# idonahum/photoVerse

Hardware: AMD Instinct MI355X
Metric: denoising steps/sec at 512x512 bs=16, 50-step loop (2 UNet fwd + CFG + DPM-Solver++ step per step) (higher is better)
Workload: dtype f16; 1 GPU; configs[1] shape timed over 96 steps instead of 50: SD-v1.5 UNet + PhotoVerse processors, 96-step loop, bs=16/GPU, 512x512 (64x64 latents), P=1, guidance 7.5, fp16; per_gpu_batch=16, global_batch=16, latent=64, parallelism=dp1 (batch-sharded, 1 all_gather), hip_graph=True, graph_branches=2

## Files before the change

### photoverse_amd/csrc/pv_gemm.hip

```cpp
#include "pv_gemm_dev.h"

namespace {

constexpr int BK = 64;
constexpr int ROW_BYTES = BK * 2;

template <int NF, int MIV = 4>
struct TileCfg {
    static constexpr int MI = MIV;
    static constexpr int BM = 2 * MI * 16;
    static constexpr int BN = NF * 32;
    static constexpr int NWAVES = 4;
    static constexpr int THREADS = NWAVES * 64;
    static constexpr int A_PER_WAVE = BM / 8 / NWAVES;
    static constexpr int STAGES = 2;
    static constexpr int A_BYTES = BM * ROW_BYTES;
    static constexpr int B_BYTES = BN * ROW_BYTES;
    static constexpr int STAGE_BYTES = A_BYTES + B_BYTES;
    static constexpr int SMEM_BYTES = STAGES * STAGE_BYTES;
    static constexpr int B_PIECES = NF * 4;
    static constexpr int B_PER_WAVE = (B_PIECES + NWAVES - 1) / NWAVES;
};

__device__ __forceinline__ float epi_act(float x, int act) {
    if (act == PV_ACT_SILU) return pv_silu(x);
    if (act == PV_ACT_QUICK_GELU) return pv_quick_gelu(x);
    if (act == PV_ACT_LEAKY_RELU) return x > 0.f ? x : 0.01f * x;
    return x;
}

__device__ __forceinline__ half8_t lds_frag(const char* base, int row, int chunk) {
    return *reinterpret_cast<const half8_t*>(base + row * ROW_BYTES + ((chunk ^ (row & 7)) << 4));
}

template <int N>
__device__ __forceinline__ void wait_vmcnt() {
    static_assert(N >= 0 && N < 64, "vmcnt is a 6-bit field");
    asm volatile("s_waitcnt vmcnt(%0)" ::"n"(N) : "memory");
}


__device__ __forceinline__ float row16_sum(float v) {
    v += __builtin_bit_cast(float, __builtin_amdgcn_update_dpp(0, __builtin_bit_cast(int, v), 0x128, 0xf, 0xf, false));
    v += __builtin_bit_cast(float, __builtin_amdgcn_update_dpp(0, __builtin_bit_cast(int, v), 0x124, 0xf, 0xf, false));
    v += __builtin_bit_cast(float, __builtin_amdgcn_update_dpp(0, __builtin_bit_cast(int, v), 0x122, 0xf, 0xf, false));
    v += __builtin_bit_cast(float, __builtin_amdgcn_update_dpp(0, __builtin_bit_cast(int, v), 0x121, 0xf, 0xf, false));
    return v;
}

template <int NF, bool CONV, bool GEGLU, bool CS = false, bool MULTI = false, int MIV = 4>
__global__ __launch_bounds__(256, MIV == 4 ? 2 : 3) void gemm_conv_kernel(const pv_gemm_params_dev p, const int tiles_n,
                                                                              const int nblk, const int order, const int tpw_arg) {
    const int tpw = MULTI ? tpw_arg : 1;
    using Cfg = TileCfg<NF, MIV>;
    static_assert(MIV == 4 || (!CS && !MULTI && !CONV), "the 64-row tile exists for plain Linear layers only");
    constexpr int BM = Cfg::BM;
    constexpr int NW = Cfg::NWAVES;
    constexpr int MI = Cfg::MI;
    constexpr int AP = Cfg::A_PER_WAVE;
    extern __shared__ __attribute__((aligned(16))) char smem[];

    const int lane = pv_lane_id();
    const int wave = pv_wave_id();
    const int bid = (order & 2) ? (int)blockIdx.x : pv_xcd_remap((int)blockIdx.x, nblk);
    const int m_fast = order & 1;
    const int tiles_m = nblk / tiles_n;
    const int tile_m = m_fast ? bid % tiles_m : bid / tiles_n;
    const int tile_n = (m_fast ? bid / tiles_m : bid % tiles_n) * tpw;
    const int m0 = tile_m * BM;
    int n0 = tile_n * Cfg::BN;

    const int cin = p.c0 + p.c1;
    const int K = p.taps * cin;
    const int nk_total = K / BK;
    const int nk_per = (nk_total + (int)gridDim.y - 1) / (int)gridDim.y;
    const int k_begin = (int)blockIdx.y * nk_per;
    const int nk = max(0, min(nk_total, k_begin + nk_per) - k_begin);

    const int lrow = lane >> 3;
    const int src_chunk = (lane & 7) ^ lrow;
    const int lane_cc2 = src_chunk * 16;
    constexpr unsigned OOB = 0x80000000u;
    const __amdgpu_buffer_rsrc_t ra0 = __builtin_amdgcn_make_buffer_rsrc(const_cast<void*>(p.a0), 0, (int)p.a0_bytes, 0x00020000);
    const __amdgpu_buffer_rsrc_t ra1 = __builtin_amdgcn_make_buffer_rsrc(const_cast<void*>(p.a1 ? p.a1 : p.a0), 0, (int)p.a1_bytes, 0x00020000);
    const __amdgpu_buffer_rsrc_t rw = __builtin_amdgcn_make_buffer_rsrc(const_cast<void*>(p.w), 0, (int)p.w_bytes, 0x00020000);
    const int hw_out = p.hout * p.wout;
    const bool fast_conv = CONV && p.stride == 1 && !p.upsample;
    const int hl = p.upsample ? p.hin * 2 : p.hin;
    const int wl = p.upsample ? p.win * 2 : p.win;
    unsigned a_off0[AP], a_off1[AP];
    unsigned a_mask[AP];
    int a_b[AP], a_y[AP], a_x[AP];
#pragma unroll
    for (int i = 0; i < AP; ++i) {
        const int m = m0 + (wave + i * NW) * 8 + lrow;
        const bool ok = m < p.M;
        if (CONV) {
            const int b = m / hw_out;
            const int rem = m - b * hw_out;
            const int y = rem / p.wout, x = rem - y * p.wout;
            a_b[i] = b; a_y[i] = y * p.stride + 1 - p.pad; a_x[i] = x * p.stride + 1 - p.pad;
            unsigned mask = 0;
#pragma unroll
            for (int t = 0; t < 9; ++t) {
                const int iy = a_y[i] + t / 3 - 1, ix = a_x[i] + t % 3 - 1;
                if (ok && iy >= 0 && iy < hl && ix >= 0 && ix < wl) mask |= 1u << t;
            }
            a_mask[i] = mask;
            const unsigned pix = (unsigned)((b * p.hin + y) * p.win + x);
            a_off0[i] = pix * (unsigned)(p.lda0 * 2) + lane_cc2;
            a_off1[i] = pix * (unsigned)(p.lda1 * 2) + lane_cc2;
        } else {
            a_mask[i] = ok ? 1u : 0u;
            a_off0[i] = ok ? (unsigned)m * (unsigned)(p.lda0 * 2) + lane_cc2 : OOB;
            a_off1[i] = ok ? (unsigned)m * (unsigned)(p.lda1 * 2) + lane_cc2 : OOB;
            a_b[i] = a_y[i] = a_x[i] = 0;
        }
    }
    unsigned w_off[Cfg::B_PER_WAVE];
#pragma unroll
    for (int i = 0; i < Cfg::B_PER_WAVE; ++i) {
        const int n = n0 + min(wave + i * NW, Cfg::B_PIECES - 1) * 8 + lrow;
        w_off[i] = (unsigned)n * (unsigned)(K * 2) + lane_cc2;
    }
    const bool b_full = (Cfg::B_PIECES % NW == 0) || (wave + (Cfg::B_PER_WAVE - 1) * NW < Cfg::B_PIECES);

    auto stage = [&](int g_local, int buf) {
        const int tn = g_local / nk;
        const int kt = k_begin + (g_local - tn * nk);
        char* sa = smem + buf * Cfg::STAGE_BYTES;
        char* sb = sa + Cfg::A_BYTES;
        const int chunk = CONV ? kt / 9 : kt;
        const int tap = CONV ? kt - chunk * 9 : 0;
        const int c = chunk * BK;
        const bool first = c < p.c0;
        const __amdgpu_buffer_rsrc_t ra = first ? ra0 : ra1;
        const int ld2 = (first ? p.lda0 : p.lda1) * 2;
        const int sc2 = (first ? c : c - p.c0) * 2;
        const int ky = tap / 3, kx = tap - ky * 3;
        const int tap_delta = ((ky - 1) * p.win + (kx - 1)) * ld2 + sc2;
#pragma unroll
        for (int i = 0; i < AP; ++i) {
            unsigned off;
            if (!CONV) {
                off = (first ? a_off0[i] : a_off1[i]) + (unsigned)sc2;
            } else if (fast_conv) {
                off = ((a_mask[i] >> tap) & 1u) ? (first ? a_off0[i] : a_off1[i]) + (unsigned)tap_delta : OOB;
            } else {
                const int iy = a_y[i] + ky - 1, ix = a_x[i] + kx - 1;
                const int py = p.upsample ? iy >> 1 : iy, px = p.upsample ? ix >> 1 : ix;
                const unsigned pix = (unsigned)((a_b[i] * p.hin + py) * p.win + px);
                off = ((a_mask[i] >> tap) & 1u) ? pix * (unsigned)ld2 + (unsigned)(sc2 + lane_cc2) : OOB;
            }
            __builtin_amdgcn_raw_ptr_buffer_load_lds(ra, PV_LDS_PTR(sa + (wave + i * NW) * 8 * ROW_BYTES), 16, (int)off, 0, 0, 0);
        }
        const unsigned wk2 = (unsigned)(tap * cin + c) * 2u + (unsigned)tn * (unsigned)(Cfg::BN * K * 2);
#pragma unroll
        for (int i = 0; i < Cfg::B_PER_WAVE; ++i) {
            if (i < Cfg::B_PER_WAVE - 1 || b_full)
                __builtin_amdgcn_raw_ptr_buffer_load_lds(rw, PV_LDS_PTR(sb + (wave + i * NW) * 8 * ROW_BYTES), 16, (int)(w_off[i] + wk2), 0, 0, 0);
        }
    };

    float4_t acc[NF][MI];
#pragma unroll
    for (int ni = 0; ni < NF; ++ni)
#pragma unroll
        for (int mi = 0; mi < MI; ++mi) acc[ni][mi] = float4_t{0.f, 0.f, 0.f, 0.f};

    const int wm = wave >> 1, wn = wave & 1;
    const int fr = lane & 15, fq = lane >> 4;

    constexpr int S = Cfg::STAGES;
    auto read_half = [&](half8_t (&xa)[MI], half8_t (&wb)[NF], int kt, int ks) {
        const char* sa = smem + (kt % S) * Cfg::STAGE_BYTES;
        const char* sb = sa + Cfg::A_BYTES;
#pragma unroll
        for (int mi = 0; mi < MI; ++mi) xa[mi] = lds_frag(sa, wm * (MI * 16) + mi * 16 + fr, ks * 4 + fq);
#pragma unroll
        for (int ni = 0; ni < NF; ++ni) wb[ni] = lds_frag(sb, wn * (NF * 16) + ni * 16 + fr, ks * 4 + fq);
    };
    auto mma_half = [&](const half8_t (&xa)[MI], const half8_t (&wb)[NF]) {
#pragma unroll
        for (int ni = 0; ni < NF; ++ni)
#pragma unroll
            for (int mi = 0; mi < MI; ++mi)
                acc[ni][mi] = __builtin_amdgcn_mfma_f32_16x16x32_f16(wb[ni], xa[mi], acc[ni][mi], 0, 0, 0);
    };

    const int T = nk * tpw;
#pragma unroll
    for (int s = 0; s < S; ++s)
        if (s < T) stage(s, s);
    if (T >= S && S == 3) {
        if (b_full) wait_vmcnt<(AP + Cfg::B_PER_WAVE) * 2>(); else wait_vmcnt<(AP + Cfg::B_PER_WAVE - 1) * 2>();
    } else if (T >= S && S == 2) {
        if (b_full) wait_vmcnt<(AP + Cfg::B_PER_WAVE)>(); else wait_vmcnt<(AP + Cfg::B_PER_WAVE - 1)>();
    } else {
        wait_vmcnt<0>();
    }
    __builtin_amdgcn_s_barrier();
    asm volatile("" ::: "memory");

    half8_t xa0[MI], wb0[NF], xa1[MI], wb1[NF];
    if (T > 0) read_half(xa0, wb0, 0, 0);
    for (int tn = 0; tn < tpw; ++tn) {
    for (int kt = 0; kt < nk; ++kt) {
        const int g = tn * nk + kt;
        read_half(xa1, wb1, g, 1);
        __builtin_amdgcn_sched_barrier(0);
        mma_half(xa0, wb0);
        __builtin_amdgcn_sched_barrier(0);
        if (g + 1 < T) {
            if (S == 3 && g + S - 1 < T) {
                if (b_full) wait_vmcnt<(AP + Cfg::B_PER_WAVE)>(); else wait_vmcnt<(AP + Cfg::B_PER_WAVE - 1)>();
            } else {
                wait_vmcnt<0>();
            }
            asm volatile("s_waitcnt lgkmcnt(0)" ::: "memory");
            __builtin_amdgcn_s_barrier();
            asm volatile("" ::: "memory");
            if (g + S < T) stage(g + S, g % S);
            __builtin_amdgcn_sched_barrier(0);
            if (kt + 1 < nk) {
                read_half(xa0, wb0, g + 1, 0);
                __builtin_amdgcn_sched_barrier(0);
            }
        }
        mma_half(xa1, wb1);
        __builtin_amdgcn_sched_barrier(0);
    }

    if (gridDim.y > 1) {
        float* slab = p.splitk_ws + (size_t)blockIdx.y * p.M * p.N;
#pragma unroll
        for (int mi = 0; mi < MI; ++mi) {
            const int m = m0 + wm * (MI * 16) + mi * 16 + fr;
            if (m >= p.M) continue;
#pragma unroll
            for (int ni = 0; ni < NF; ++ni) {
                const int n = n0 + wn * (NF * 16) + ni * 16 + fq * 4;
                *reinterpret_cast<float4_t*>(slab + (size_t)m * p.N + n) = acc[ni][mi];
            }
        }
        return;
    }
    const int nbase = n0 + wn * (NF * 16) + fq * 4;
    if (GEGLU) {
        float4_t bv[NF / 2], bg[NF / 2];
#pragma unroll
        for (int q = 0; q < NF / 2; ++q) {
            bv[q] = p.bias ? *reinterpret_cast<const float4_t*>(p.bias + nbase + (2 * q) * 16) : float4_t{0.f, 0.f, 0.f, 0.f};
            bg[q] = p.bias ? *reinterpret_cast<const float4_t*>(p.bias + nbase + (2 * q + 1) * 16) : float4_t{0.f, 0.f, 0.f, 0.f};
        }
#pragma unroll
        for (int mi = 0; mi < MI; ++mi) {
            const int m = m0 + wm * (MI * 16) + mi * 16 + fr;
            if (m >= p.M) continue;
            unsigned pk[NF / 2][2];
#pragma unroll
            for (int q = 0; q < NF / 2; ++q) {
                const float4_t v = acc[2 * q][mi] + bv[q], g = acc[2 * q + 1][mi] + bg[q];
                pk[q][0] = __builtin_bit_cast(unsigned, half2_t{(half_t)(v[0] * pv_gelu_erf(g[0])), (half_t)(v[1] * pv_gelu_erf(g[1]))});
                pk[q][1] = __builtin_bit_cast(unsigned, half2_t{(half_t)(v[2] * pv_gelu_erf(g[2])), (half_t)(v[3] * pv_gelu_erf(g[3]))});
            }
            half_t* orow = reinterpret_cast<half_t*>(p.out) + (size_t)m * p.ldc + (n0 >> 1) + wn * (NF * 8);
            static_assert(!GEGLU || NF == 4, "GEGLU epilogue pairs the two value|gate fragment pairs of a wave");
            {
                const auto r0 = __builtin_amdgcn_permlane16_swap(pk[0][0], pk[1][0], false, false);
                const auto r1 = __builtin_amdgcn_permlane16_swap(pk[0][1], pk[1][1], false, false);
                const unsigned a0 = r0[0], b0 = r0[1], a1 = r1[0], b1 = r1[1];
                const int col = (fq & 1) ? 16 + (fq - 1) * 4 : fq * 4;
                typedef unsigned uint4_t __attribute__((ext_vector_type(4)));
                *reinterpret_cast<uint4_t*>(orow + col) = uint4_t{a0, a1, b0, b1};
            }
        }
    } else {
        float4_t bias_v[NF];
#pragma unroll
        for (int ni = 0; ni < NF; ++ni)
            bias_v[ni] = p.bias ? *reinterpret_cast<const float4_t*>(p.bias + nbase + ni * 16) : float4_t{0.f, 0.f, 0.f, 0.f};
        constexpr int RB = MULTI ? 2 : MI;
        half4_t res[NF][MI];
        if (p.residual && !MULTI) {
#pragma unroll
            for (int mi = 0; mi < MI; ++mi) {
                const int m = min(m0 + wm * (MI * 16) + mi * 16 + fr, p.M - 1);
#pragma unroll
                for (int ni = 0; ni < NF; ++ni)
                    res[ni][mi] = *reinterpret_cast<const half4_t*>(reinterpret_cast<const half_t*>(p.residual) + (size_t)m * p.ldr + nbase + ni * 16);
            }
        }
        const bool want_cs = CS && p.colstats != nullptr && !p.out_f32;
        float4_t cs[NF], cq[NF];
#pragma unroll
        for (int ni = 0; ni < NF; ++ni) cs[ni] = cq[ni] = float4_t{0.f, 0.f, 0.f, 0.f};
#pragma unroll
        for (int mi = 0; mi < MI; ++mi) {
            if (MULTI && p.residual && mi % RB == 0) {
#pragma unroll
                for (int m2 = mi; m2 < mi + RB; ++m2) {
                    const int mm = min(m0 + wm * (MI * 16) + m2 * 16 + fr, p.M - 1);
#pragma unroll
                    for (int ni = 0; ni < NF; ++ni)
                        res[ni][m2] = *reinterpret_cast<const half4_t*>(reinterpret_cast<const half_t*>(p.residual) + (size_t)mm * p.ldr + nbase + ni * 16);
                }
            }
            const int m = m0 + wm * (MI * 16) + mi * 16 + fr;
            if (m >= p.M) continue;
            const float* radd = p.rowadd ? p.rowadd + (size_t)(m / hw_out) * p.rowadd_ld + nbase : nullptr;
            unsigned pk[NF][2];
#pragma unroll
            for (int ni = 0; ni < NF; ++ni) {
                float4_t v = acc[ni][mi] + bias_v[ni];
                if (radd) v += *reinterpret_cast<const float4_t*>(radd + ni * 16);
                if (p.act) {
#pragma unroll
                    for (int r = 0; r < 4; ++r) v[r] = epi_act(v[r], p.act);
                }
                if (p.residual) {
#pragma unroll
                    for (int r = 0; r < 4; ++r) v[r] += (float)res[ni][mi][r];
                }
                if (p.out_f32) {
                    *reinterpret_cast<float4_t*>(reinterpret_cast<float*>(p.out) + (size_t)m * p.ldc + nbase + ni * 16) = v;
                } else {
                    const half4_t hv = half4_t{(half_t)v[0], (half_t)v[1], (half_t)v[2], (half_t)v[3]};
                    pk[ni][0] = __builtin_bit_cast(unsigned, half2_t{hv[0], hv[1]});
                    pk[ni][1] = __builtin_bit_cast(unsigned, half2_t{hv[2], hv[3]});
                    if (want_cs) {
#pragma unroll
                        for (int r = 0; r < 4; ++r) {
                            const float f = (float)hv[r];
                            cs[ni][r] += f;
                            cq[ni][r] += f * f;
                        }
                    }
                }
            }
            if (!p.out_f32) {
                half_t* orow = reinterpret_cast<half_t*>(p.out) + (size_t)m * p.ldc + n0 + wn * (NF * 16);
#pragma unroll
                for (int q = 0; q < NF / 2; ++q) {
                    const auto r0 = __builtin_amdgcn_permlane16_swap(pk[2 * q][0], pk[2 * q + 1][0], false, false);
                    const auto r1 = __builtin_amdgcn_permlane16_swap(pk[2 * q][1], pk[2 * q + 1][1], false, false);
                    const unsigned a0 = r0[0], b0 = r0[1], a1 = r1[0], b1 = r1[1];
                    const int col = (fq & 1) ? (2 * q + 1) * 16 + (fq - 1) * 4 : (2 * q) * 16 + fq * 4;
                    typedef unsigned uint4_t __attribute__((ext_vector_type(4)));
                    *reinterpret_cast<uint4_t*>(orow + col) = uint4_t{a0, a1, b0, b1};
                }
                if (NF & 1) {
                    typedef unsigned uint2_t __attribute__((ext_vector_type(2)));
                    *reinterpret_cast<uint2_t*>(orow + (NF - 1) * 16 + fq * 4) = uint2_t{pk[NF - 1][0], pk[NF - 1][1]};
                }
            }
        }
        if (want_cs && m0 + wm * (MI * 16) < p.M) {
#pragma unroll
            for (int ni = 0; ni < NF; ++ni)
#pragma unroll
                for (int r = 0; r < 4; ++r) {
                    cs[ni][r] = row16_sum(cs[ni][r]);
                    cq[ni][r] = row16_sum(cq[ni][r]);
                }
            if (fr == 0) {
                float* dst = p.colstats + ((size_t)(m0 / 64 + wm) * 2) * p.N + nbase;
#pragma unroll
                for (int ni = 0; ni < NF; ++ni) {
                    *reinterpret_cast<float4_t*>(dst + ni * 16) = cs[ni];
                    *reinterpret_cast<float4_t*>(dst + p.N + ni * 16) = cq[ni];
                }
            }
        }
    }
    if (tn + 1 < tpw) {
#pragma unroll
        for (int ni = 0; ni < NF; ++ni)
#pragma unroll
            for (int mi = 0; mi < MI; ++mi) acc[ni][mi] = float4_t{0.f, 0.f, 0.f, 0.f};
        n0 += Cfg::BN;
        read_half(xa0, wb0, (tn + 1) * nk, 0);
        __builtin_amdgcn_sched_barrier(0);
    }
    }
}

__global__ __launch_bounds__(256) void splitk_reduce_kernel(const pv_gemm_params_dev p, const int splits) {
    __shared__ float red[2][16][64];
    const int cq = threadIdx.x & 15, rg = threadIdx.x >> 4;
    const int n = (int)blockIdx.x * 64 + cq * 4;
    const int mb = (int)blockIdx.y * 64 + rg * 4;
    const bool ncol = n < p.N;
    float4_t cs = float4_t{0.f, 0.f, 0.f, 0.f}, cq2 = float4_t{0.f, 0.f, 0.f, 0.f};
    if (ncol) {
        const float4_t bias = p.bias ? *reinterpret_cast<const float4_t*>(p.bias + n) : float4_t{0.f, 0.f, 0.f, 0.f};
#pragma unroll
        for (int r = 0; r < 4; ++r) {
            const int m = mb + r;
            if (m >= p.M) break;
            float4_t v = float4_t{0.f, 0.f, 0.f, 0.f};
            for (int s = 0; s < splits; ++s) v += *reinterpret_cast<const float4_t*>(p.splitk_ws + ((size_t)s * p.M + m) * p.N + n);
            v += bias;
            if (p.rowadd) v += *reinterpret_cast<const float4_t*>(p.rowadd + (size_t)(m / (p.hout * p.wout)) * p.rowadd_ld + n);
            if (p.act) {
#pragma unroll
                for (int j = 0; j < 4; ++j) v[j] = epi_act(v[j], p.act);
            }
            if (p.residual) {
                const half4_t rr = *reinterpret_cast<const half4_t*>(reinterpret_cast<const half_t*>(p.residual) + (size_t)m * p.ldr + n);
#pragma unroll
                for (int j = 0; j < 4; ++j) v[j] += (float)rr[j];
            }
            if (p.out_f32) {
                *reinterpret_cast<float4_t*>(reinterpret_cast<float*>(p.out) + (size_t)m * p.ldc + n) = v;
            } else {
                half4_t o;
#pragma unroll
                for (int j = 0; j < 4; ++j) {
                    o[j] = (half_t)v[j];
                    const float f = (float)o[j];
                    cs[j] += f;
                    cq2[j] += f * f;
                }
                *reinterpret_cast<half4_t*>(reinterpret_cast<half_t*>(p.out) + (size_t)m * p.ldc + n) = o;
            }
        }
    }
    if (p.colstats == nullptr) return;
#pragma unroll
    for (int j = 0; j < 4; ++j) {
        red[0][rg][cq * 4 + j] = cs[j];
        red[1][rg][cq * 4 + j] = cq2[j];
    }
    __syncthreads();
    if (threadIdx.x < 128) {
        const int which = threadIdx.x >> 6, col = threadIdx.x & 63;
        float a = 0.f;
#pragma unroll
        for (int g = 0; g < 16; ++g) a += red[which][g][col];
        const int nn = (int)blockIdx.x * 64 + col;
        if (nn < p.N) p.colstats[((size_t)blockIdx.y * 2 + which) * p.N + nn] = a;
    }
}

template <int NF, bool CONV, bool GEGLU, bool CS = false, bool MULTI = false, int MIV = 4>
int launch(const pv_gemm_params_dev& p, hipStream_t stream, int tpw = 1) {
    using Cfg = TileCfg<NF, MIV>;
    if (pv_gemm_probe) {
        const int splits_ = (!GEGLU && p.splitk > 1 && p.splitk_ws) ? p.splitk : 1;
        snprintf(pv_gemm_probe->name, sizeof(pv_gemm_probe->name), "gemm_conv_kernel<%d, %s, %s, %s, %s, %d>", NF, CONV ? "true" : "false", GEGLU ? "true" : "false",
                 CS ? "true" : "false", MULTI ? "true" : "false", MIV);
        pv_gemm_probe->wgs = (long)(((p.M + Cfg::BM - 1) / Cfg::BM) * (p.N / Cfg::BN) / tpw) * splits_;
        return 0;
    }
    static bool attr_set_dev[64] = {};
    int dev_id = 0;
    (void)hipGetDevice(&dev_id);
    bool& attr_set = attr_set_dev[dev_id & 63];
    auto kern = gemm_conv_kernel<NF, CONV, GEGLU, CS, MULTI, MIV>;
    if (!attr_set) {
        hipError_t e = hipFuncSetAttribute(reinterpret_cast<const void*>(kern), hipFuncAttributeMaxDynamicSharedMemorySize,
                                           Cfg::SMEM_BYTES);
        if (e != hipSuccess) return (int)e;
        attr_set = true;
    }
    const int tiles_m = (p.M + Cfg::BM - 1) / Cfg::BM;
    const int tiles_n = p.N / Cfg::BN;
    const int nblk = tiles_m * tiles_n;
    const size_t wbytes = (size_t)p.N * p.taps * (p.c0 + p.c1) * 2;
    static const int order_env = getenv("PV_TILE_ORDER") ? atoi(getenv("PV_TILE_ORDER")) : -1;
    const int m_fast = order_env >= 0 ? order_env : ((wbytes > (3u << 20)) && tiles_n >= 8 ? 1 : 0);
    const int splits = (!GEGLU && p.splitk > 1 && p.splitk_ws) ? p.splitk : 1;
    hipLaunchKernelGGL(kern, dim3(nblk / tpw, splits), dim3(Cfg::THREADS), Cfg::SMEM_BYTES, stream, p, tiles_n / tpw, nblk / tpw, m_fast, tpw);
    if (splits > 1) return pv_gemm_splitk_reduce_launch(p, splits, stream);
    return PV_CHECK_LAUNCH();
}

template <int NF>
int choose_tpw(const pv_gemm_params_dev& p) {
    static const int tpw_env = getenv("PV_GEMM_TPW") ? atoi(getenv("PV_GEMM_TPW")) : 0;
    if (p.taps != 1 || (p.splitk > 1 && p.splitk_ws)) return 1;
    const int tiles_n = p.N / (NF * 32), nk = (p.c0 + p.c1) / BK;
    const long nblk = (long)((p.M + 127) / 128) * tiles_n;
    if (tpw_env > 0) return tiles_n % tpw_env == 0 ? tpw_env : 1;
    for (int c = 8; c >= 2; --c)
        if (tiles_n % c == 0 && nk <= 5 && nblk / c >= 1024) return c;
    return 1;
}

template <int NF, bool CONV, bool GEGLU>
int dispatch(const pv_gemm_params_dev& p, hipStream_t stream) {
    if constexpr (!CONV && GEGLU) {
        const int tpw = choose_tpw<NF>(p);
        if (tpw > 1) return launch<NF, false, true, false, true>(p, stream, tpw);
    }
    if constexpr (!GEGLU) {
        if (p.colstats && !(p.splitk > 1 && p.splitk_ws)) return launch<NF, CONV, false, true>(p, stream);
    }
    if constexpr (!CONV && !GEGLU) {
        static const int mi2_env = getenv("PV_GEMM_MI2") ? atoi(getenv("PV_GEMM_MI2")) : 512;
        const long tiles128 = (long)((p.M + 127) / 128) * (p.N / (NF * 32));
        if (!(p.splitk > 1 && p.splitk_ws) && tiles128 < mi2_env) return launch<NF, false, false, false, false, 2>(p, stream);
    }
    return launch<NF, CONV, GEGLU>(p, stream);
}

}

int pv_gemm_splitk_reduce_launch(const pv_gemm_params_dev& p, int splits, hipStream_t stream) {
    hipLaunchKernelGGL(splitk_reduce_kernel, dim3((unsigned)((p.N + 63) / 64), (unsigned)((p.M + 63) / 64)), dim3(256), 0, stream, p, splits);
    return PV_CHECK_LAUNCH();
}

thread_local pv_launch_probe* pv_gemm_probe = nullptr;

extern "C" int pv_gemm_conv(const pv_gemm_params* pp, void* stream_);

extern "C" int pv_gemm_conv_kernel_info(const pv_gemm_params* pp, char* name, int32_t name_len, int64_t* workgroups) {
    if (!pp || !name || name_len <= 0) return (int)hipErrorInvalidValue;
    pv_launch_probe probe;
    probe.name[0] = 0;
    probe.wgs = 0;
    pv_gemm_probe = &probe;
    const int rc = pv_gemm_conv(pp, nullptr);
    pv_gemm_probe = nullptr;
    if (rc != 0) return rc;
    if ((int)strlen(probe.name) >= name_len) return (int)hipErrorInvalidValue;
    strcpy(name, probe.name);
    if (workgroups) *workgroups = probe.wgs;
    return 0;
}

extern "C" int pv_gemm_conv(const pv_gemm_params* pp, void* stream_) {
    pv_gemm_params_dev p;
    static_cast<pv_gemm_params&>(p) = *pp;
    hipStream_t stream = reinterpret_cast<hipStream_t>(stream_);
    const int cin = p.c0 + p.c1;
    if (p.M <= 0 || p.N <= 0 || cin <= 0 || (cin % 64) || (p.c0 % 64) || (p.taps != 1 && p.taps != 9) || p.act == PV_ACT_GELU || p.splitk < 0 || p.splitk > 16 ||
        !p.a0 || !p.w || !p.out || (p.c1 && !p.a1) || p.hout * p.wout <= 0)
        return (int)hipErrorInvalidValue;
    if (p.colstats && (p.geglu || p.out_f32)) return (int)hipErrorInvalidValue;
    if (p.taps == 9 && !(p.pad == 1 || (p.pad == 0 && p.stride == 2 && !p.upsample))) return (int)hipErrorInvalidValue;
    {
        const size_t a_rows = p.taps == 9 ? (size_t)p.batch * p.hin * p.win : (size_t)p.M;
        const size_t b0 = ((a_rows - 1) * p.lda0 + p.c0) * 2, b1 = p.c1 ? ((a_rows - 1) * p.lda1 + p.c1) * 2 : 0;
        const size_t bw = (size_t)p.N * p.taps * cin * 2;
        if (b0 >= (1ull << 31) || b1 >= (1ull << 31) || bw >= (1ull << 31)) return (int)hipErrorInvalidValue;
        p.a0_bytes = (uint32_t)b0;
        p.a1_bytes = (uint32_t)b1;
        p.w_bytes = (uint32_t)bw;
    }
    if (p.geglu && (p.taps != 1 || (p.N % 128))) return (int)hipErrorInvalidValue;
    if (p.a_norm && (p.taps != 9 || (p.a_norm_act != PV_ACT_NONE && p.a_norm_act != PV_ACT_SILU))) return (int)hipErrorInvalidValue;
    {
        const int rc = pv_conv_big_launch(p, stream);
        if (rc >= 0) return rc;
        if (rc == -2 || p.a_norm) return (int)hipErrorInvalidValue;
    }
    if (p.ln_rowsum) return (int)hipErrorInvalidValue;
    if (p.geglu) return dispatch<4, false, true>(p, stream);
    const bool conv = p.taps == 9;
    if (p.N % 160 == 0) return conv ? dispatch<5, true, false>(p, stream) : dispatch<5, false, false>(p, stream);
    if (p.N % 128 == 0) return conv ? dispatch<4, true, false>(p, stream) : dispatch<4, false, false>(p, stream);
    return (int)hipErrorInvalidValue;
}
```

### photoverse_amd/csrc/pv_gemm_dev.h

```cpp
#pragma once
#include "pv_common.h"

struct pv_gemm_params_dev : pv_gemm_params {
    uint32_t a0_bytes, a1_bytes, w_bytes;
};

__attribute__((visibility("hidden"))) int pv_conv_big_launch(const pv_gemm_params_dev& p, hipStream_t stream);


__attribute__((visibility("hidden"))) int pv_gemm_splitk_reduce_launch(const pv_gemm_params_dev& p, int splits, hipStream_t stream);


struct pv_launch_probe {
    char name[160];
    long wgs;
};
extern thread_local pv_launch_probe* pv_gemm_probe;
```

### photoverse_amd/csrc/pv_rowgemm.hip

```cpp
#include "pv_common.h"
#include <stdlib.h>

namespace {

constexpr int RG_K = 320;
constexpr int RG_CHUNK = 160;
constexpr int RG_TILE = RG_CHUNK * 128;
constexpr int RG_SLOTS = 4;
constexpr int RG_SMEM = RG_SLOTS * RG_TILE;

struct pv_rowgemm_params_dev : pv_row_gemm_params {
    uint32_t w_bytes;
};

template <int N>
__device__ __forceinline__ void rg_wait_vmcnt() {
    static_assert(N >= 0 && N < 64, "vmcnt is a 6-bit field");
    asm volatile("s_waitcnt vmcnt(%0)" ::"n"(N) : "memory");
}

template <bool GEGLU>
__global__ __launch_bounds__(256, 2) void row_gemm_kernel(const pv_rowgemm_params_dev p) {
    constexpr int C = RG_K;
    constexpr int KK = C / 32;
    constexpr int KT = C / 64;
    constexpr int NFC = RG_CHUNK / 16;
    typedef unsigned uint4_t __attribute__((ext_vector_type(4)));
    typedef unsigned uint2_t __attribute__((ext_vector_type(2)));
    extern __shared__ __attribute__((aligned(16))) char smem[];

    const int lane = pv_lane_id(), wave = pv_wave_id();
    const int fr = lane & 15, g = lane >> 4;
    const int m0 = (int)blockIdx.x * 128;
    const int rows_here = min(128, p.M - m0);
    const int n_chunks = p.N / RG_CHUNK;
    const int NT = n_chunks * KT;

    const __amdgpu_buffer_rsrc_t rw = __builtin_amdgcn_make_buffer_rsrc(const_cast<void*>(p.w), 0, (int)p.w_bytes, 0x00020000);
    const __amdgpu_buffer_rsrc_t rx = __builtin_amdgcn_make_buffer_rsrc(const_cast<half_t*>(reinterpret_cast<const half_t*>(p.x)) + (size_t)m0 * p.ld_x, 0,
                                                                        rows_here * p.ld_x * 2, 0x00020000);
    const int ld_o = p.ld_out;
    const __amdgpu_buffer_rsrc_t ro = __builtin_amdgcn_make_buffer_rsrc(reinterpret_cast<half_t*>(p.out) + (size_t)m0 * ld_o, 0, rows_here * ld_o * 2, 0x00020000);

    const int lrow = lane >> 3;
    const unsigned w_lane_off = (unsigned)lrow * (unsigned)(C * 2) + (unsigned)(((lane & 7) ^ lrow) << 4);
    const unsigned piece_off = w_lane_off + (unsigned)(wave * 8) * (unsigned)(C * 2);
    auto issue_stage = [&](int t) {
        const int nc = t / KT, kt = t - nc * KT;
        char* dst = smem + (t & (RG_SLOTS - 1)) * RG_TILE;
        const int soff = nc * RG_CHUNK * (C * 2) + kt * 128;
#pragma unroll
        for (int i = 0; i < 5; ++i)
            __builtin_amdgcn_raw_ptr_buffer_load_lds(rw, PV_LDS_PTR(dst + (wave + 4 * i) * 1024), 16, (int)piece_off, soff + i * 32 * (C * 2), 0, 0);
    };
    auto wg_barrier = [&]() {
        asm volatile("s_waitcnt lgkmcnt(0)" ::: "memory");
        __builtin_amdgcn_s_barrier();
        asm volatile("" ::: "memory");
    };

    half8_t xf[KK][2];
    int mrow[2];
#pragma unroll
    for (int qi = 0; qi < 2; ++qi) {
        mrow[qi] = wave * 32 + qi * 16 + fr;
        const int off = mrow[qi] * p.ld_x * 2 + g * 16;
#pragma unroll
        for (int kk = 0; kk < KK; ++kk) xf[kk][qi] = __builtin_bit_cast(half8_t, __builtin_amdgcn_raw_buffer_load_b128(rx, off, kk * 64, 0));
    }
    issue_stage(0);
    issue_stage(1);
    if (p.x_norm) {
        const float* tab = p.x_norm + (size_t)(m0 / p.rows_per_image) * 2 * C + g * 8;
#pragma unroll
        for (int kk = 0; kk < KK; ++kk) {
            const float4_t s0 = *reinterpret_cast<const float4_t*>(tab + kk * 32), s1 = *reinterpret_cast<const float4_t*>(tab + kk * 32 + 4);
            const float4_t h0 = *reinterpret_cast<const float4_t*>(tab + C + kk * 32), h1 = *reinterpret_cast<const float4_t*>(tab + C + kk * 32 + 4);
#pragma unroll
            for (int qi = 0; qi < 2; ++qi)
#pragma unroll
                for (int j = 0; j < 8; ++j) xf[kk][qi][j] = (half_t)((float)xf[kk][qi][j] * (j < 4 ? s0[j & 3] : s1[j & 3]) + (j < 4 ? h0[j & 3] : h1[j & 3]));
        }
    }
    if (p.ln) {
        typedef _Float16 h2_t __attribute__((ext_vector_type(2)));
        const h2_t ones = h2_t{(half_t)1.0f, (half_t)1.0f};
#pragma unroll
        for (int qi = 0; qi < 2; ++qi) {
            float sum = 0.f;
#pragma unroll
            for (int kk = 0; kk < KK; ++kk)
#pragma unroll
                for (int j = 0; j < 4; ++j) sum = __builtin_amdgcn_fdot2(h2_t{xf[kk][qi][2 * j], xf[kk][qi][2 * j + 1]}, ones, sum, false);
            const float mean = pv_quad_sum(sum) * (1.0f / (float)C);
            const half_t mh = (half_t)mean;
            const h2_t nm = h2_t{(half_t)(-mh), (half_t)(-mh)};
            float sq = 0.f;
#pragma unroll
            for (int kk = 0; kk < KK; ++kk)
#pragma unroll
                for (int j = 0; j < 4; ++j) {
                    const h2_t d = h2_t{xf[kk][qi][2 * j], xf[kk][qi][2 * j + 1]} + nm;
                    sq = __builtin_amdgcn_fdot2(d, d, sq, false);
                }
            const float dm = mean - (float)mh;
            const float var = pv_quad_sum(sq) * (1.0f / (float)C) - dm * dm;
            const float rstd = rsqrtf(fmaxf(var, 0.f) + p.ln_eps);
            const float nmr = -mean * rstd;
#pragma unroll
            for (int kk = 0; kk < KK; ++kk)
#pragma unroll
                for (int j = 0; j < 8; ++j) xf[kk][qi][j] = (half_t)fmaf((float)xf[kk][qi][j], rstd, nmr);
        }
    }
    rg_wait_vmcnt<0>();

    const int ring_lane[2] = {fr * 128 + ((g ^ (fr & 7)) << 4), fr * 128 + (((4 + g) ^ (fr & 7)) << 4)};
    const int pcol = (g & 1) ? 16 + (g - 1) * 4 : g * 4;
    constexpr int OUT_PER_CHUNK = GEGLU ? RG_CHUNK / 2 : RG_CHUNK;
    constexpr int STORES = GEGLU ? 6 : 10;

    float4_t acc[NFC][2];
    for (int it = 0; it < n_chunks / 2; ++it) {
        const int t0 = it * (2 * KT);
#pragma unroll
        for (int j = 0; j < 2 * KT; ++j) {
            const int t = t0 + j;
            const int kt = j % KT;
            const int nc = 2 * it + j / KT;
            if ((j & 1) == 0) {
                const bool stores_since = (j == 6) || (j == 0 && it > 0);
                if (t >= 2) {
                    if (stores_since) rg_wait_vmcnt<STORES>(); else rg_wait_vmcnt<0>();
                }
                wg_barrier();
                if (t + 2 < NT) issue_stage(t + 2);
                if (t + 3 < NT) issue_stage(t + 3);
            }
            if (kt == 0) {
#pragma unroll
                for (int i = 0; i < NFC; ++i)
                    acc[i][0] = acc[i][1] = p.bias ? *reinterpret_cast<const float4_t*>(p.bias + nc * RG_CHUNK + i * 16 + g * 4) : float4_t{0.f, 0.f, 0.f, 0.f};
            }
            const char* slot = smem + (t & (RG_SLOTS - 1)) * RG_TILE;
#pragma unroll
            for (int ks = 0; ks < 2; ++ks) {
                const char* base = slot + ring_lane[ks];
#pragma unroll
                for (int i = 0; i < NFC; ++i) {
                    const half8_t a = *reinterpret_cast<const half8_t*>(base + i * 2048);
#pragma unroll
                    for (int qi = 0; qi < 2; ++qi) acc[i][qi] = __builtin_amdgcn_mfma_f32_16x16x32_f16(a, xf[2 * kt + ks][qi], acc[i][qi], 0, 0, 0);
                }
            }
            if (kt == KT - 1) {
                const int ocol0 = nc * OUT_PER_CHUNK;
#pragma unroll
                for (int qi = 0; qi < 2; ++qi) {
                    const int ooff = mrow[qi] * ld_o * 2 + ocol0 * 2;
                    unsigned pk[GEGLU ? NFC / 2 : NFC][2];
                    if (GEGLU) {
#pragma unroll
                        for (int q = 0; q < NFC / 2; ++q) {
                            const float4_t v = acc[2 * q][qi], gt = acc[2 * q + 1][qi];
                            pk[q][0] = __builtin_bit_cast(unsigned, half2_t{(half_t)(v[0] * pv_gelu_erf(gt[0])), (half_t)(v[1] * pv_gelu_erf(gt[1]))});
                            pk[q][1] = __builtin_bit_cast(unsigned, half2_t{(half_t)(v[2] * pv_gelu_erf(gt[2])), (half_t)(v[3] * pv_gelu_erf(gt[3]))});
                        }
                    } else {
#pragma unroll
                        for (int i = 0; i < NFC; ++i) {
                            const float4_t v = acc[i][qi];
                            pk[i][0] = __builtin_bit_cast(unsigned, half2_t{(half_t)v[0], (half_t)v[1]});
                            pk[i][1] = __builtin_bit_cast(unsigned, half2_t{(half_t)v[2], (half_t)v[3]});
                        }
                    }
                    constexpr int NOUT = GEGLU ? NFC / 2 : NFC;
#pragma unroll
                    for (int q = 0; q < NOUT / 2; ++q) {
                        const auto v0 = __builtin_amdgcn_permlane16_swap(pk[2 * q][0], pk[2 * q + 1][0], false, false);
                        const auto v1 = __builtin_amdgcn_permlane16_swap(pk[2 * q][1], pk[2 * q + 1][1], false, false);
                        const unsigned sa0 = v0[0], sb0 = v0[1], sa1 = v1[0], sb1 = v1[1];
                        __builtin_amdgcn_raw_buffer_store_b128(uint4_t{sa0, sa1, sb0, sb1}, ro, ooff + pcol * 2 + q * 64, 0, 0);
                        asm volatile("s_nop 1" ::: "memory");
                    }
                    if (NOUT & 1)
                        __builtin_amdgcn_raw_buffer_store_b64(uint2_t{pk[NOUT - 1][0], pk[NOUT - 1][1]}, ro, ooff + g * 8 + (NOUT - 1) * 32, 0, 0);
                }
                __builtin_amdgcn_sched_barrier(0);
            }
        }
    }
}

}

extern "C" int pv_row_gemm(const pv_row_gemm_params* pp, void* stream) {
    pv_rowgemm_params_dev p;
    static_cast<pv_row_gemm_params&>(p) = *pp;
    if (!p.x || !p.w || !p.out || p.M <= 0 || p.K != RG_K || p.N <= 0 || (p.N % (2 * RG_CHUNK)) || (p.ld_x % 8) || (p.ld_out % 8) || p.ld_x < RG_K ||
        p.ld_out < (p.geglu ? p.N / 2 : p.N) || (p.x_norm && (p.ln || p.rows_per_image <= 0 || (p.rows_per_image % 128) || (p.M % p.rows_per_image))))
        return (int)hipErrorInvalidValue;
    if ((size_t)p.N * RG_K * 2 >= (1ull << 31)) return (int)hipErrorInvalidValue;
    p.w_bytes = (uint32_t)p.N * RG_K * 2;
    static bool attr_set_dev[64][2] = {};
    int dev_id = 0;
    (void)hipGetDevice(&dev_id);
    bool& attr_set = attr_set_dev[dev_id & 63][p.geglu ? 1 : 0];
    auto kern = p.geglu ? row_gemm_kernel<true> : row_gemm_kernel<false>;
    if (!attr_set) {
        hipError_t e = hipFuncSetAttribute(reinterpret_cast<const void*>(kern), hipFuncAttributeMaxDynamicSharedMemorySize, RG_SMEM);
        if (e != hipSuccess) return (int)e;
        attr_set = true;
    }
    hipLaunchKernelGGL(kern, dim3((unsigned)((p.M + 127) / 128)), dim3(256), RG_SMEM, (hipStream_t)stream, p);
    return PV_CHECK_LAUNCH();
}
```

Baseline: 33.78 denoising steps/s (bs=16 per GPU, summed over GPUs).

## Add row-resident K=320 residual GEMM kernel with fused column stats

Adds a specialized kernel for 1x1 GEMMs with K=320, N=320, a residual add and optional column statistics (sum and sum of squares for a following norm). It keeps each 128-row A tile in registers and streams weights through an LDS ring, folding bias, residual and stats into the epilogue. It is tried before the generic conv/GEMM path, so that path's tiling and load overhead is skipped for these shapes in the 320-channel stage. The risk is that this kernel is slower than the existing tuned path, and the hand-written permlane and DPP layout logic could contain correctness bugs.

```diff
diff --git a/photoverse_amd/csrc/pv_gemm.hip b/photoverse_amd/csrc/pv_gemm.hip
--- a/photoverse_amd/csrc/pv_gemm.hip
+++ b/photoverse_amd/csrc/pv_gemm.hip
@@ -1,4 +1,8 @@
 #include "pv_gemm_dev.h"
+
+#ifndef PV_K320_RES_ROW
+#define PV_K320_RES_ROW 1
+#endif
 
 namespace {
 
@@ -552,6 +556,12 @@
     }
     if (p.geglu && (p.taps != 1 || (p.N % 128))) return (int)hipErrorInvalidValue;
     if (p.a_norm && (p.taps != 9 || (p.a_norm_act != PV_ACT_NONE && p.a_norm_act != PV_ACT_SILU))) return (int)hipErrorInvalidValue;
+#if PV_K320_RES_ROW
+    {
+        const int rc = pv_row_res_launch(p, stream);
+        if (rc >= 0) return rc;
+    }
+#endif
     {
         const int rc = pv_conv_big_launch(p, stream);
         if (rc >= 0) return rc;
diff --git a/photoverse_amd/csrc/pv_gemm_dev.h b/photoverse_amd/csrc/pv_gemm_dev.h
--- a/photoverse_amd/csrc/pv_gemm_dev.h
+++ b/photoverse_amd/csrc/pv_gemm_dev.h
@@ -8,6 +8,9 @@
 __attribute__((visibility("hidden"))) int pv_conv_big_launch(const pv_gemm_params_dev& p, hipStream_t stream);
 
 
+__attribute__((visibility("hidden"))) int pv_row_res_launch(const pv_gemm_params_dev& p, hipStream_t stream);
+
+
 __attribute__((visibility("hidden"))) int pv_gemm_splitk_reduce_launch(const pv_gemm_params_dev& p, int splits, hipStream_t stream);
 
 
diff --git a/photoverse_amd/csrc/pv_rowgemm.hip b/photoverse_amd/csrc/pv_rowgemm.hip
--- a/photoverse_amd/csrc/pv_rowgemm.hip
+++ b/photoverse_amd/csrc/pv_rowgemm.hip
@@ -1,4 +1,5 @@
-#include "pv_common.h"
+#include "pv_gemm_dev.h"
+#include <stdio.h>
 #include <stdlib.h>
 
 namespace {
@@ -192,6 +193,246 @@
     }
 }
 
+
+struct pv_rowres_params_dev {
+    const void* x;
+    const void* w;
+    const float* bias;
+    const void* residual;
+    void* out;
+    float* colstats;
+    int32_t M, ld_x, ld_r, ld_out;
+};
+
+__device__ __forceinline__ float rr_row16_sum(float v) {
+    v += __builtin_bit_cast(float, __builtin_amdgcn_update_dpp(0, __builtin_bit_cast(int, v), 0x128, 0xf, 0xf, false));
+    v += __builtin_bit_cast(float, __builtin_amdgcn_update_dpp(0, __builtin_bit_cast(int, v), 0x124, 0xf, 0xf, false));
+    v += __builtin_bit_cast(float, __builtin_amdgcn_update_dpp(0, __builtin_bit_cast(int, v), 0x122, 0xf, 0xf, false));
+    v += __builtin_bit_cast(float, __builtin_amdgcn_update_dpp(0, __builtin_bit_cast(int, v), 0x121, 0xf, 0xf, false));
+    return v;
+}
+
+template <bool CS>
+__global__ __launch_bounds__(256, 2) void row_res_gemm_kernel(const pv_rowres_params_dev p) {
+    constexpr int C = RG_K;
+    constexpr int N = 320;
+    constexpr int KT = C / 64;
+    constexpr int NFC = RG_CHUNK / 16;
+    constexpr int NT = 2 * KT;
+    constexpr int STORES = 10;
+    typedef unsigned uint4_t __attribute__((ext_vector_type(4)));
+    extern __shared__ __attribute__((aligned(16))) char smem[];
+
+    const int lane = pv_lane_id(), wave = pv_wave_id();
+    const int fr = lane & 15, g = lane >> 4;
+    const int m0 = (int)blockIdx.x * 128;
+    const int rows_here = min(128, p.M - m0);
+
+    const __amdgpu_buffer_rsrc_t rw = __builtin_amdgcn_make_buffer_rsrc(const_cast<void*>(p.w), 0, N * C * 2, 0x00020000);
+    const __amdgpu_buffer_rsrc_t rx = __builtin_amdgcn_make_buffer_rsrc(const_cast<half_t*>(reinterpret_cast<const half_t*>(p.x)) + (size_t)m0 * p.ld_x, 0,
+                                                                        ((rows_here - 1) * p.ld_x + C) * 2, 0x00020000);
+    const __amdgpu_buffer_rsrc_t rr = __builtin_amdgcn_make_buffer_rsrc(const_cast<half_t*>(reinterpret_cast<const half_t*>(p.residual)) + (size_t)m0 * p.ld_r, 0,
+                                                                        ((rows_here - 1) * p.ld_r + N) * 2, 0x00020000);
+    const __amdgpu_buffer_rsrc_t rb = __builtin_amdgcn_make_buffer_rsrc(const_cast<float*>(p.bias), 0, p.bias ? N * 4 : 0, 0x00020000);
+    const __amdgpu_buffer_rsrc_t ro = __builtin_amdgcn_make_buffer_rsrc(reinterpret_cast<half_t*>(p.out) + (size_t)m0 * p.ld_out, 0,
+                                                                        ((rows_here - 1) * p.ld_out + N) * 2, 0x00020000);
+
+    const int lrow = lane >> 3;
+    const unsigned w_lane_off = (unsigned)lrow * (unsigned)(C * 2) + (unsigned)(((lane & 7) ^ lrow) << 4);
+    const unsigned piece_off = w_lane_off + (unsigned)(wave * 8) * (unsigned)(C * 2);
+    auto issue_stage = [&](int t) {
+        const int nc = t / KT, kt = t - nc * KT;
+        char* dst = smem + (t & (RG_SLOTS - 1)) * RG_TILE;
+        const int soff = nc * RG_CHUNK * (C * 2) + kt * 128;
+#pragma unroll
+        for (int i = 0; i < 5; ++i)
+            __builtin_amdgcn_raw_ptr_buffer_load_lds(rw, PV_LDS_PTR(dst + (wave + 4 * i) * 1024), 16, (int)piece_off, soff + i * 32 * (C * 2), 0, 0);
+    };
+    auto wg_barrier = [&]() {
+        asm volatile("s_waitcnt lgkmcnt(0)" ::: "memory");
+        __builtin_amdgcn_s_barrier();
+        asm volatile("" ::: "memory");
+    };
+
+    half8_t xf[C / 32][2];
+    int mrow[2];
+#pragma unroll
+    for (int qi = 0; qi < 2; ++qi) {
+        mrow[qi] = wave * 32 + qi * 16 + fr;
+        const int off = mrow[qi] * p.ld_x * 2 + g * 16;
+#pragma unroll
+        for (int kk = 0; kk < C / 32; ++kk) xf[kk][qi] = __builtin_bit_cast(half8_t, __builtin_amdgcn_raw_buffer_load_b128(rx, off, kk * 64, 0));
+    }
+    issue_stage(0);
+    issue_stage(1);
+
+    const int pcol = (g & 1) ? 16 + (g - 1) * 4 : g * 4;
+    auto res_pair = [&](const uint4_t L, float4_t& lo, float4_t& hi) {
+        const auto r0 = __builtin_amdgcn_permlane16_swap(L[0], L[2], false, false);
+        const auto r1 = __builtin_amdgcn_permlane16_swap(L[1], L[3], false, false);
+        const half2_t a0 = __builtin_bit_cast(half2_t, (unsigned)r0[0]), a1 = __builtin_bit_cast(half2_t, (unsigned)r1[0]);
+        const half2_t b0 = __builtin_bit_cast(half2_t, (unsigned)r0[1]), b1 = __builtin_bit_cast(half2_t, (unsigned)r1[1]);
+        lo = float4_t{(float)a0[0], (float)a0[1], (float)a1[0], (float)a1[1]};
+        hi = float4_t{(float)b0[0], (float)b0[1], (float)b1[0], (float)b1[1]};
+    };
+
+    float4_t acc[NFC][2];
+    {
+        uint4_t r0[2][NFC / 2];
+#pragma unroll
+        for (int qi = 0; qi < 2; ++qi) {
+            const int roff = mrow[qi] * p.ld_r * 2 + pcol * 2;
+#pragma unroll
+            for (int q = 0; q < NFC / 2; ++q) r0[qi][q] = __builtin_amdgcn_raw_buffer_load_b128(rr, roff + q * 64, 0, 0);
+        }
+#pragma unroll
+        for (int i = 0; i < NFC; ++i) acc[i][0] = __builtin_bit_cast(float4_t, __builtin_amdgcn_raw_buffer_load_b128(rb, g * 16 + i * 64, 0, 0));
+#pragma unroll
+        for (int qi = 1; qi >= 0; --qi)
+#pragma unroll
+            for (int q = 0; q < NFC / 2; ++q) {
+                float4_t lo, hi;
+                res_pair(r0[qi][q], lo, hi);
+                acc[2 * q][qi] = acc[2 * q][0] + lo;
+                acc[2 * q + 1][qi] = acc[2 * q + 1][0] + hi;
+            }
+    }
+    rg_wait_vmcnt<0>();
+
+    const int ring_lane[2] = {fr * 128 + ((g ^ (fr & 7)) << 4), fr * 128 + (((4 + g) ^ (fr & 7)) << 4)};
+    const bool valid[2] = {mrow[0] < rows_here, mrow[1] < rows_here};
+    uint4_t res1[2][NFC / 2];
+    float cshold[2][NFC / 2];
+
+#pragma unroll
+    for (int j = 0; j < NT; ++j) {
+        const int kt = j % KT, nc = j / KT;
+        if ((j & 1) == 0) {
+            if (j >= 2) {
+                if (j == 6) rg_wait_vmcnt<STORES>(); else rg_wait_vmcnt<0>();
+            }
+            wg_barrier();
+            if (j + 2 < NT) issue_stage(j + 2);
+            if (j + 3 < NT) issue_stage(j + 3);
+            if (j == NT - 2) {
+#pragma unroll
+                for (int qi = 0; qi < 2; ++qi) {
+                    const int roff = mrow[qi] * p.ld_r * 2 + (RG_CHUNK + pcol) * 2;
+#pragma unroll
+                    for (int q = 0; q < NFC / 2; ++q) res1[qi][q] = __builtin_amdgcn_raw_buffer_load_b128(rr, roff + q * 64, 0, 0);
+                }
+                __builtin_amdgcn_sched_barrier(0);
+            }
+        }
+        if (j == KT) {
+#pragma unroll
+            for (int i = 0; i < NFC; ++i)
+                acc[i][0] = acc[i][1] = __builtin_bit_cast(float4_t, __builtin_amdgcn_raw_buffer_load_b128(rb, RG_CHUNK * 4 + g * 16 + i * 64, 0, 0));
+        }
+        const char* slot = smem + (j & (RG_SLOTS - 1)) * RG_TILE;
+#pragma unroll
+        for (int ks = 0; ks < 2; ++ks) {
+            const char* base = slot + ring_lane[ks];
+#pragma unroll
+            for (int i = 0; i < NFC; ++i) {
+                const half8_t a = *reinterpret_cast<const half8_t*>(base + i * 2048);
+#pragma unroll
+                for (int qi = 0; qi < 2; ++qi) acc[i][qi] = __builtin_amdgcn_mfma_f32_16x16x32_f16(a, xf[2 * kt + ks][qi], acc[i][qi], 0, 0, 0);
+            }
+        }
+        if (j >= NT - 2) __builtin_amdgcn_sched_barrier(0);
+        if (kt == KT - 1) {
+#pragma unroll
+            for (int q = 0; q < NFC / 2; ++q) {
+                unsigned pk[2][2][2];
+#pragma unroll
+                for (int qi = 0; qi < 2; ++qi) {
+                    float4_t va = acc[2 * q][qi], vb = acc[2 * q + 1][qi];
+                    if (nc == 1) {
+                        float4_t lo, hi;
+                        res_pair(res1[qi][q], lo, hi);
+                        va += lo;
+                        vb += hi;
+                    }
+                    pk[qi][0][0] = __builtin_bit_cast(unsigned, half2_t{(half_t)va[0], (half_t)va[1]});
+                    pk[qi][0][1] = __builtin_bit_cast(unsigned, half2_t{(half_t)va[2], (half_t)va[3]});
+                    pk[qi][1][0] = __builtin_bit_cast(unsigned, half2_t{(half_t)vb[0], (half_t)vb[1]});
+                    pk[qi][1][1] = __builtin_bit_cast(unsigned, half2_t{(half_t)vb[2], (half_t)vb[3]});
+                    if (CS) asm("" : "+v"(pk[qi][0][0]), "+v"(pk[qi][0][1]), "+v"(pk[qi][1][0]), "+v"(pk[qi][1][1]));
+                    const auto v0 = __builtin_amdgcn_permlane16_swap(pk[qi][0][0], pk[qi][1][0], false, false);
+                    const auto v1 = __builtin_amdgcn_permlane16_swap(pk[qi][0][1], pk[qi][1][1], false, false);
+                    const unsigned sa0 = v0[0], sb0 = v0[1], sa1 = v1[0], sb1 = v1[1];
+                    __builtin_amdgcn_raw_buffer_store_b128(uint4_t{sa0, sa1, sb0, sb1}, ro, mrow[qi] * p.ld_out * 2 + nc * RG_CHUNK * 2 + pcol * 2 + q * 64, 0, 0);
+                    asm volatile("s_nop 1" ::: "memory");
+                }
+                if (CS) {
+                    float hold = 0.f;
+#pragma unroll
+                    for (int e = 0; e < 2; ++e)
+#pragma unroll
+                        for (int r = 0; r < 4; ++r) {
+                            const half2_t h0 = __builtin_bit_cast(half2_t, pk[0][e][r >> 1]), h1 = __builtin_bit_cast(half2_t, pk[1][e][r >> 1]);
+                            const float f0 = valid[0] ? (float)h0[r & 1] : 0.f, f1 = valid[1] ? (float)h1[r & 1] : 0.f;
+                            const float sm = rr_row16_sum(f0 + f1), sq = rr_row16_sum(f0 * f0 + f1 * f1);
+                            hold = fr == e * 8 + r ? sm : hold;
+                            hold = fr == e * 8 + 4 + r ? sq : hold;
+                        }
+                    asm volatile("" : "+v"(hold));
+                    cshold[nc][q] = hold;
+                    __builtin_amdgcn_sched_barrier(0);
+                }
+            }
+            __builtin_amdgcn_sched_barrier(0);
+        }
+    }
+    if (CS) {
+        float* part = reinterpret_cast<float*>(smem + 2 * RG_TILE);
+        const int ccol = ((fr >> 2) & 1) * N + (fr >> 3) * 16 + g * 4 + (fr & 3);
+#pragma unroll
+        for (int nc = 0; nc < 2; ++nc)
+#pragma unroll
+            for (int q = 0; q < NFC / 2; ++q) part[wave * (2 * N) + ccol + nc * RG_CHUNK + q * 32] = cshold[nc][q];
+        wg_barrier();
+#pragma unroll
+        for (int k = 0; k < 5; ++k) {
+            const int e = (int)threadIdx.x + 256 * k;
+            const int b = e >= 2 * N ? 1 : 0, c = e - b * (2 * N);
+            if (m0 + 64 * b < p.M) p.colstats[(size_t)(m0 / 64 + b) * (2 * N) + c] = part[(2 * b) * (2 * N) + c] + part[(2 * b + 1) * (2 * N) + c];
+        }
+    }
+}
+
+}
+
+int pv_row_res_launch(const pv_gemm_params_dev& p, hipStream_t stream) {
+    if (p.taps != 1 || p.c0 != RG_K || p.c1 != 0 || p.N != 320 || !p.residual || p.geglu || p.out_f32 || p.act != 0 || p.rowadd || p.splitk > 1 || p.ln_rowsum ||
+        p.a_norm)
+        return -1;
+    if ((p.lda0 % 8) || (p.ldc % 8) || (p.ldr % 8) || p.lda0 < RG_K || p.ldc < 320 || p.ldr < 320) return -1;
+    if ((((size_t)p.M - 1) * p.ldc + 320) * 2 >= (1ull << 31) || (((size_t)p.M - 1) * p.ldr + 320) * 2 >= (1ull << 31)) return -1;
+    if ((reinterpret_cast<uintptr_t>(p.a0) | reinterpret_cast<uintptr_t>(p.w) | reinterpret_cast<uintptr_t>(p.residual) | reinterpret_cast<uintptr_t>(p.out)) & 15) return -1;
+    const bool cs = p.colstats != nullptr;
+    const unsigned wgs = (unsigned)((p.M + 127) / 128);
+    if (pv_gemm_probe) {
+        snprintf(pv_gemm_probe->name, sizeof(pv_gemm_probe->name), "row_res_gemm_kernel<%s>", cs ? "true" : "false");
+        pv_gemm_probe->wgs = (long)wgs;
+        return 0;
+    }
+    pv_rowres_params_dev d;
+    d.x = p.a0; d.w = p.w; d.bias = p.bias; d.residual = p.residual; d.out = p.out; d.colstats = p.colstats;
+    d.M = p.M; d.ld_x = p.lda0; d.ld_r = p.ldr; d.ld_out = p.ldc;
+    static bool attr_set_dev[64][2] = {};
+    int dev_id = 0;
+    (void)hipGetDevice(&dev_id);
+    bool& attr_set = attr_set_dev[dev_id & 63][cs ? 1 : 0];
+    auto kern = cs ? row_res_gemm_kernel<true> : row_res_gemm_kernel<false>;
+    if (!attr_set) {
+        hipError_t e = hipFuncSetAttribute(reinterpret_cast<const void*>(kern), hipFuncAttributeMaxDynamicSharedMemorySize, RG_SMEM);
+        if (e != hipSuccess) return (int)e;
+        attr_set = true;
+    }
+    hipLaunchKernelGGL(kern, dim3(wgs), dim3(256), RG_SMEM, (hipStream_t)stream, d);
+    return PV_CHECK_LAUNCH();
 }
 
 extern "C" int pv_row_gemm(const pv_row_gemm_params* pp, void* stream) {
```

Result: no change. 33.88 denoising steps/s (bs=16 per GPU, summed over GPUs), median of 6 (+0.3%).
